# Audio-WestlakeU/FS-EEND

Hardware: AMD Instinct MI355X
Metric: audio frames/sec (T=500 chunks) (higher is better)
Workload: dtype bf16

## Files before the change

fs-eend_amd/csrc/api.hip:

```cpp
#include "../../include/eend_hip.h"
#include "kernels.h"
#include <stdlib.h>
#include <string.h>

namespace {
GemmParams base_params(const void* A, int lda, const void* W, int ldw, const float* bias, int M, int N, int K) {
    GemmParams p;
    memset(&p, 0, sizeof(p));
    p.A = A; p.lda = lda; p.W = W; p.ldw = ldw; p.bias = bias;
    p.M = M; p.N = N; p.K = K; p.ldo = N; p.Tp = 64; p.H = 4; p.dh = 64; p.C = 1;
    p.alpha = 1.0f; p.eps = 1e-5f; p.conv_cin = 64; p.conv_pad = 0; p.drop.scale = 1.0f;
#ifdef EEND_GEMM_ABLATE
    const char* d = getenv("EEND_GEMM_DBG");
    p.dbg = d ? atoi(d) : 0;
#endif
    return p;
}
}

extern "C" {

int eend_abi_version(void) { return 5; }

int eend_bn_cast_pad_f16(const float* x, const float* bn_weight, const float* bn_bias, const float* bn_mean,
// ... 207 lines not shown
    memset(&p, 0, sizeof(p));
    p.A = A; p.lda = lda; p.wstream = wstream; p.bo = bo; p.g1 = g1; p.be1 = be1; p.eps1 = eps1; p.res32 = res; p.res16 = res_f16;
    p.b1 = b1; p.b2 = b2; p.alpha = 1.0f; p.gamma = g2; p.beta = be2; p.eps = eps2; p.out32 = out_f32; p.out16 = out_f16;
    p.M = M; p.F = F;
    return ffn_stream_chunked(p, 1, 1, FFN_EPI_RES_LN, (hipStream_t)stream);
}

int eend_attnout_ffn_stream_lo_f16(const void* A, int lda, const void* wstream, const float* bo, const float* res, const float* g1,
                                   const float* be1, float eps1, const float* b1, const float* b2, const float* g2, const float* be2,
                                   float eps2, float* out_f32, void* out_f16, void* out_lo_f16, int M, int F, void* stream) {
    if (!res) return EEND_EINVAL;
    FfnStreamParams p;
    memset(&p, 0, sizeof(p));
    p.A = A; p.lda = lda; p.wstream = wstream; p.bo = bo; p.g1 = g1; p.be1 = be1; p.eps1 = eps1; p.res32 = res; p.wo_lo = 1;
    p.b1 = b1; p.b2 = b2; p.alpha = 1.0f; p.gamma = g2; p.beta = be2; p.eps = eps2; p.out32 = out_f32; p.out16 = out_f16; p.out16lo = out_lo_f16;
    p.M = M; p.F = F;
    return ffn_stream_chunked(p, 1, 1, FFN_EPI_RES_LN, (hipStream_t)stream);
}

int eend_conv_stream_elems(int ktaps) { return (int)eend_conv_stream_nelems(ktaps); }

int eend_conv_stream_ok(int cin, int ktaps, int pad) { return eend_conv_stream_supported(cin, ktaps, pad); }

int eend_conv_stream_pack_f16(const void* Wr, void* stream_out, int ktaps, void* stream) {
    return eend_launch_conv_stream_pack(Wr, stream_out, ktaps, (hipStream_t)stream);
}

int eend_conv1d_l2norm_stream_f16(const void* X, const void* wstream, const float* bias, const int* ilens, float* out_f32,
                                  void* out_f16, int nseq, int Tp, int ktaps, int pad, void* stream) {
    ConvStreamParams p;
    memset(&p, 0, sizeof(p));
    p.X = X; p.wstream = wstream; p.bias = bias; p.ilens = ilens; p.out32 = out_f32; p.out16 = out_f16; p.nseq = nseq; p.Tp = Tp;
    p.ktaps = ktaps; p.pad = pad;
    return eend_launch_conv_stream(p, (hipStream_t)stream);
}

int eend_encoder_input_ok(int Fin, int Tp, int ldw) { return eend_encin_supported(Fin, Tp, ldw); }

int eend_encoder_input_f16(const float* const* x_ptrs, const int* lens, float pad_value, const float* bn_w, const float* bn_b,
                           const float* bn_mean, const float* bn_var, float bn_eps, const void* W_f16, int ldw, const float* bias,
                           const float* gamma, const float* beta, float eps, float* out_f32, void* out_f16, int B, int T, int Tp,
                           int Fin, void* stream) {
    EncInParams p;
    memset(&p, 0, sizeof(p));
    p.x_ptrs = x_ptrs; p.lens = lens; p.pad_value = pad_value; p.bn_w = bn_w; p.bn_b = bn_b; p.bn_mean = bn_mean; p.bn_var = bn_var;
    p.bn_eps = bn_eps; p.W = W_f16; p.ldw = ldw; p.bias = bias; p.gamma = gamma; p.beta = beta; p.eps = eps; p.out32 = out_f32;
    p.out16 = out_f16; p.B = B; p.T = T; p.Tp = Tp; p.Fin = Fin;
    return eend_launch_encin(p, (hipStream_t)stream);
}

int eend_dec_stream_elems(int F) { return F >= 64 && F % 64 == 0 && F <= 2048 ? (int)eend_dec_stream_nelems(F) : 0; }

int eend_dec_stream_ok(int C, int Tp) { return eend_dec_stream_supported(C, Tp); }

int eend_dec_stream_pack_f16(const void* Wo1, const void* W_in, const void* Wo2, const void* W1, const void* W2, void* stream_out, int F,
                             void* stream) {
    return eend_launch_dec_stream_pack(Wo1, W_in, Wo2, W1, W2, stream_out, F, (hipStream_t)stream);
}

int eend_attnout_spk_ffn_stream_f16(const void* A, int lda, const void* wstream, const float* bo1, const void* res_f16, const float* g11,
                                    const float* be11, float eps11, const float* b_in, const float* bo2, const float* g21, const float* be21,
                                    float eps21, const float* b1, const float* b2, const float* g22, const float* be22, float eps22,
                                    void* out_f16, int B, int C, int Tp, int F, float scale, void* stream) {
    DecStreamParams p;
    memset(&p, 0, sizeof(p));
    p.A = A; p.lda = lda; p.wstream = wstream; p.bo1 = bo1; p.g11 = g11; p.be11 = be11; p.eps11 = eps11; p.res16 = res_f16; p.bin = b_in;
// ... 429 lines not shown
```

fs-eend_amd/csrc/conv_stream.hip:

```cpp
#include "common.h"
#include "kernels.h"
#include "wstream.h"

namespace {

constexpr int NR = 4;
constexpr int NF = 8;
constexpr int TM = 128, WM = 64;
constexpr int SLOT = STREAM_ITEM;
constexpr int NSLOT = 5;
constexpr int MAXTAPS = 24;
constexpr int XROWS = TM + MAXTAPS;
constexpr int L_RING = 0;
constexpr int L_X = NSLOT * SLOT;
constexpr int L_VEC = L_X + XROWS * 512;
constexpr int L_SS = L_VEC + 1024;
constexpr int SMEM = L_SS + 1024;
constexpr int NB = 8, PD = 4;
constexpr int INFL = 4 * (NSLOT - 3);

__global__ void conv_stream_pack_kernel(const _Float16* __restrict__ Wr, _Float16* __restrict__ out, int ktaps) {
    const long total = (long)ktaps * 8 * 1024;
    for (long t = (long)blockIdx.x * blockDim.x + threadIdx.x; t < total; t += (long)gridDim.x * blockDim.x) {
        const int item = (int)(t >> 10), w = (int)(t & 1023), i = w >> 6, l = w & 63, f = l & 15, g = l >> 4;
        const int tau = item >> 3, kc = item & 7;
        const _Float16* src = Wr + (size_t)((i >> 3) * 128 + (f >> 2) * 32 + (i & 7) * 4 + (f & 3)) * (ktaps * 256) + tau * 256 + kc * 32 + g * 8;
        _Float16* dst = out + t * 8;
#pragma unroll
        for (int e = 0; e < 8; ++e) dst[e] = src[e];
    }
}

__global__ __launch_bounds__(256, 1)
void conv_stream_kernel(const ConvStreamParams p) {
    const int S = p.ktaps * 8;
    const int TPS = (p.Tp + TM - 1) / TM;
    const int ntiles = p.nseq * TPS;
    const int xrows = TM + p.ktaps - 1;

    int tid = threadIdx.x;
    asm volatile("" : "+v"(tid));
    int lane = tid & 63;
    const int wave = __builtin_amdgcn_readfirstlane(tid >> 6);
    int frow = lane & 15, g = lane >> 4;

    WeightRing<NSLOT, L_RING> ring(p.wstream, S, wave, lane);
    ring.prime();
    float* vb = (float*)(smem + L_VEC);
    vb[tid] = p.bias[tid];

    auto stage_x = [&](int tile) __attribute__((always_inline)) {
        const int seq = __builtin_amdgcn_readfirstlane(tile / TPS), t0 = (tile - seq * TPS) * TM;
        int len = p.ilens[seq];
        len = len < p.Tp ? len : p.Tp;
        const __amdgpu_buffer_rsrc_t rx = __builtin_amdgcn_make_buffer_rsrc((void*)((const char*)p.X + (size_t)seq * p.Tp * 512), 0, len * 512, 0x00020000);
        const int npc = (xrows + 1) >> 1;
        for (int pc = wave; pc < npc; pc += 4) {
            const int r = 2 * pc + (lane >> 5);
            const int off = (t0 - p.pad + r) * 512 + (((lane & 31) ^ (r & 7)) << 4);
            __builtin_amdgcn_raw_ptr_buffer_load_lds(rx, (lds_char*)(smem + L_X + pc * 1024), 16, off, 0, 0, 0);
        }
    };

    const int rg = wave >> 1, nh = wave & 1;
    f16x8 wf[NB];
    f32x4 acc[NF][NR];
    bool cold = true;
    for (int tile = blockIdx.x; tile < ntiles; tile += gridDim.x) {
        asm volatile("" : "+v"(tid));
        lane = tid & 63; frow = lane & 15; g = lane >> 4;
        ring.set_lane(lane);
        const int seq = __builtin_amdgcn_readfirstlane(tile / TPS), t0 = (tile - seq * TPS) * TM;
        asm volatile("s_waitcnt lgkmcnt(0)\n\ts_barrier" ::: "memory");
        stage_x(tile);
        asm volatile("s_waitcnt vmcnt(0)\n\ts_barrier" ::: "memory");
#pragma unroll
        for (int i = 0; i < NF; ++i) {
            const f32x4 b4 = *(const f32x4*)(vb + nh * 128 + g * 32 + i * 4);
#pragma unroll
            for (int j = 0; j < NR; ++j) acc[i][j] = b4;
        }
        const char* xl = smem + L_X;
        auto read_x = [&](int q, f16x8 (&xo)[NR]) __attribute__((always_inline)) {
            const int tau = q >> 3, kc = q & 7;
#pragma unroll
            for (int j = 0; j < NR; ++j) {
                const int r = rg * WM + j * 16 + frow + tau;
                xo[j] = *(const f16x8*)(xl + r * 512 + (((kc * 4 + g) ^ (r & 7)) << 4));
            }
        };
        f16x8 xf[NR], xn[NR];
        read_x(0, xf);
        for (int q = 0; q < S; ++q) {
            if (q > 0) {
                wait_vm<INFL>();
                __builtin_amdgcn_s_barrier();
            }
            const char* wc = smem + L_RING + ring.slot * SLOT + nh * (NF * 1024) + lane * 16;
            const char* wn = smem + L_RING + ring.next_slot() * SLOT + nh * (NF * 1024) + lane * 16;
            const int sd = ring.refill_slot();
            if (cold) {
                sfor<PD>([&](auto Q) __attribute__((always_inline)) { wf[decltype(Q)::value % NB] = *(const f16x8*)(wc + decltype(Q)::value * 1024); });
                cold = false;
            }
            sfor<NF>([&](auto PI) __attribute__((always_inline)) {
                constexpr int pi = decltype(PI)::value;
                const f16x8 w = wf[pi % NB];
#pragma unroll
                for (int j = 0; j < NR; ++j) acc[pi][j] = __builtin_amdgcn_mfma_f32_16x16x32_f16(w, xf[j], acc[pi][j], 0, 0, 0);
                if constexpr (pi + PD < NF) wf[(pi + PD) % NB] = *(const f16x8*)(wc + (pi + PD) * 1024);
                else wf[(pi + PD) % NB] = *(const f16x8*)(wn + (pi + PD - NF) * 1024);
                if constexpr (pi < 4) ring.piece<pi>(sd);
                if constexpr (pi == 2) { if (q + 1 < S) read_x(q + 1, xn); }
                __builtin_amdgcn_sched_barrier(0);
            });
#pragma unroll
            for (int j = 0; j < NR; ++j) xf[j] = xn[j];
            ring.advance();
            ring.rotate();
        }
        asm volatile("s_waitcnt lgkmcnt(0)\n\ts_barrier" ::: "memory");
        asm volatile("" : "+v"(tid));
        lane = tid & 63; frow = lane & 15; g = lane >> 4;
        float* ssl = (float*)(smem + L_SS);
        float ss[NR];
#pragma unroll
        for (int j = 0; j < NR; ++j) {
            f32x2 sq2 = f32x2{0.f, 0.f};
#pragma unroll
            for (int i = 0; i < NF; ++i) {
                const f32x2 x0 = f32x2{acc[i][j][0], acc[i][j][1]}, x1 = f32x2{acc[i][j][2], acc[i][j][3]};
                sq2 = x1 * x1 + (x0 * x0 + sq2);
            }
            ss[j] = wave_g_allreduce_add(sq2[0] + sq2[1]);
            if (g == 0) ssl[(rg * WM + j * 16 + frow) * 2 + nh] = ss[j];
        }
        asm volatile("s_waitcnt lgkmcnt(0)\n\ts_barrier" ::: "memory");
        char* st = smem + L_X + wave * 4096;
        const int tlim = p.Tp - t0;
        sfor<NR>([&](auto J) __attribute__((always_inline)) {
            constexpr int j = decltype(J)::value;
            const float rinv = 1.0f / __builtin_sqrtf(ss[j] + ssl[(rg * WM + j * 16 + frow) * 2 + (nh ^ 1)]);
            if (p.inv_norm) { const int rr = rg * WM + j * 16 + frow; if (g == 0 && nh == 0 && rr < tlim) p.inv_norm[(size_t)seq * p.Tp + t0 + rr] = rinv; }
#pragma unroll
            for (int half = 0; half < 2; ++half) {
                const int rb = rg * WM + j * 16 + half * 8;
                if ((frow >> 3) == half) {
#pragma unroll
                    for (int e = 0; e < 4; ++e) {
                        f16x8 o;
#pragma unroll
                        for (int q = 0; q < 8; ++q) o[q] = to_f16_sat(acc[e * 2 + (q >> 2)][j][q & 3] * rinv);
                        *(f16x8*)(st + (frow & 7) * 256 + (((g * 4 + e) ^ (frow & 7)) << 4)) = o;
                    }
                }
                wave_lds_sync();
#pragma unroll
                for (int ps = 0; ps < 2; ++ps) {
                    const int rr = lane >> 3, cc = (lane & 7) + 8 * ps;
                    const f16x8 v = *(const f16x8*)(st + rr * 256 + ((cc ^ rr) << 4));
                    if (rb + rr < tlim) *(f16x8*)((_Float16*)p.out16 + ((size_t)seq * p.Tp + t0 + rb + rr) * 256 + nh * 128 + cc * 8) = v;
                }
                wave_lds_sync();
                if ((frow >> 3) == half) {
#pragma unroll
                    for (int e = 0; e < 8; ++e) *(f32x4*)(st + (frow & 7) * 512 + (((g * 8 + e) ^ (frow & 7)) << 4)) = acc[e][j] * rinv;
                }
                wave_lds_sync();
#pragma unroll
                for (int ps = 0; ps < 4; ++ps) {
                    const int rr = lane >> 3, cc = (lane & 7) + 8 * ps;
                    const f32x4 v = *(const f32x4*)(st + rr * 512 + ((cc ^ rr) << 4));
                    if (rb + rr < tlim) *(f32x4*)(p.out32 + ((size_t)seq * p.Tp + t0 + rb + rr) * 256 + nh * 128 + cc * 4) = v;
                }
                wave_lds_sync();
            }
        });
    }
    asm volatile("s_waitcnt vmcnt(0)" ::: "memory");
}

}

long eend_conv_stream_nelems(int ktaps) { return (long)ktaps * 8 * (SLOT / 2); }

int eend_conv_stream_supported(int cin, int ktaps, int pad) { return cin == 256 && ktaps >= 1 && ktaps <= MAXTAPS && pad >= 0 && pad < ktaps; }

int eend_launch_conv_stream_pack(const void* Wr, void* out, int ktaps, hipStream_t stream) {
    if (!Wr || !out || ktaps < 1 || ktaps > MAXTAPS) return EEND_EINVAL;
    hipLaunchKernelGGL(conv_stream_pack_kernel, dim3(ktaps * 8 * 4), dim3(256), 0, stream, (const _Float16*)Wr, (_Float16*)out, ktaps);
    return hipGetLastError() == hipSuccess ? EEND_OK : EEND_ELAUNCH;
}

int eend_launch_conv_stream(const ConvStreamParams& p, hipStream_t stream) {
    if (!p.X || !p.wstream || !p.bias || !p.ilens || !p.out32 || !p.out16 || p.nseq <= 0 || p.Tp <= 0 || !eend_conv_stream_supported(256, p.ktaps, p.pad) ||
        (long)p.Tp * 512 >= (1L << 31))
        return EEND_EINVAL;
    return stream_launch<conv_stream_kernel>(p, SMEM, p.nseq * ((p.Tp + TM - 1) / TM), eend_cu_count(), stream);
}
```

fs-eend_amd/csrc/kernels.h:

```cpp
#pragma once
#include <hip/hip_runtime.h>
#include <stdint.h>
#include "../../include/eend_hip.h"
#include "common.h"

enum GemmEpilogue {
    EPI_PLAIN_F16 = 0,
    EPI_PLAIN_RELU_F16 = 1,
    EPI_QK_HEADS = 2,
    EPI_VT_HEADS = 3,
    EPI_RES_LN = 4,
    EPI_L2NORM = 5,
    EPI_CONVERT = 6,
    EPI_RES_SCALE = 7,
    EPI_RES_SCALE_LN16 = 8,
    EPI_PLAIN_SWISH_F16 = 9,
    EPI_GLU_F16 = 10,
    EPI_QK_HEADS_F16 = 11,
    EPI_KTVT_HEADS_F16 = 12,
    EPI_PLAIN_BF16 = 13,
    EPI_MASK_BF16 = 14,
    EPI_F32_ROWMASK = 15,
    EPI_RES_LN_TRAIN = 16,
    EPI_L2NORM_TRAIN = 17,
// ... 313 lines not shown
    const float* be11;
    float eps11;
    const void* res16;
    const float* bin;
    const float* bo2;
    const float* g21;
    const float* be21;
    float eps21;
    const float* b1;
    const float* b2;
    const float* g22;
    const float* be22;
    float eps22;
    void* out16;
    int B, C, Tp, F;
    float scale;
};
long eend_dec_stream_nelems(int F);
int eend_dec_stream_supported(int C, int Tp);
int eend_launch_dec_stream_pack(const void* Wo1, const void* Win, const void* Wo2, const void* W1, const void* W2, void* out, int F,
                                hipStream_t stream);
int eend_launch_dec_stream(const DecStreamParams& p, hipStream_t stream);
int eend_launch_convert_fanout_rows(const void* E, const void* W1, const float* pc, float* out32, void* out16, int B, int Tp, int C,
                                    hipStream_t stream);
struct ConvStreamParams {
    const void* X;
    const void* wstream;
    const float* bias;
    const int* ilens;
    float* out32;
    void* out16;
    float* inv_norm;
    int nseq, Tp, ktaps, pad;
};
long eend_conv_stream_nelems(int ktaps);
int eend_conv_stream_supported(int cin, int ktaps, int pad);
int eend_launch_conv_stream_pack(const void* Wr, void* out, int ktaps, hipStream_t stream);
int eend_launch_conv_stream(const ConvStreamParams& p, hipStream_t stream);
struct EncInParams {
    const float* const* x_ptrs;
    const int* lens;
    float pad_value;
    const float *bn_w, *bn_b, *bn_mean, *bn_var;
    float bn_eps;
    const void* W;
    int ldw;
    const float *bias, *gamma, *beta;
    float eps;
    float* out32;
    void* out16;
    int B, T, Tp, Fin;
};
int eend_encin_supported(int Fin, int Tp, int ldw);
int eend_launch_encin(const EncInParams& p, hipStream_t stream);
int eend_launch_convert_fanout_f32(const float* emb, const float* W, int ldw, const float* pc, float* out32, void* out16, void* out16lo,
                                   int B, int Tp, int C, hipStream_t stream);
int eend_launch_attn_causal_full(const AttnParams& p, hipStream_t stream);

enum ProjKind { PROJ_ROWMAJOR = 0, PROJ_HEADS = 1, PROJ_HEADS_T = 2, PROJ_HEADS_BOTH = 3 };
struct ProjParams {
    const void* X;
    const void* W;
    const float* bias;
    int M, N, ldx, Tp, H;
    int kind[4];
    int is_bf16[4];
    void* out[4];
    void* out2[4];
    int ld[4];
};
// ... 156 lines not shown
```

fs-eend_amd/fs_model.py:

```python
import copy
import math
from typing import List, Optional, Sequence

import torch
import torch.nn as nn
from torch import Tensor

from . import ops
from .lib import EendHipError

_D_SUPPORTED = 256
_H_SUPPORTED = 4


class PositionalEncoding(nn.Module):

    def __init__(self, d_model, dropout=0.1, max_len=5000):
        super().__init__()
        self.dropout = nn.Dropout(p=dropout)
        pe = torch.zeros(max_len, d_model)
        position = torch.arange(0, max_len, dtype=torch.float).unsqueeze(1)
        div_term = torch.exp(torch.arange(0, d_model, 2).float() * (-math.log(10000.0) / d_model))
        pe[:, 0::2] = torch.sin(position * div_term)
        pe[:, 1::2] = torch.cos(position * div_term)
        self.register_buffer("pe", pe.unsqueeze(0))


class TransformerEncoder(nn.Module):

    def __init__(self, encoder_layer, num_layers, norm=None):
        super().__init__()
        self.layers = nn.ModuleList([copy.deepcopy(encoder_layer) for _ in range(num_layers)])
        self.num_layers = num_layers
        self.norm = norm
# ... 162 lines not shown
        P = {}
        enc = self.enc
        Fin = enc.in_size
        Fin_pad = (Fin + 63) // 64 * 64
        w = torch.zeros(enc.n_units, Fin_pad, dtype=torch.float16, device=dev)
        w[:, :Fin] = enc.encoder.weight.detach().to(torch.float16)
        P["enc.in.w"], P["enc.in.b"] = w, _f32(enc.encoder.bias)
        P["enc.in.g"], P["enc.in.beta"] = _f32(enc.encoder_norm.weight), _f32(enc.encoder_norm.bias)
        P["enc.in.eps"] = enc.encoder_norm.eps
        P["bn"] = tuple(_f32(t) for t in (enc.bn.weight, enc.bn.bias, enc.bn.running_mean, enc.bn.running_var))
        P["bn.eps"] = enc.bn.eps
        P["Fin_pad"] = Fin_pad
        layers = []
        for l in enc.transformer_encoder.layers:
            layers.append(dict(
                in_w=_f16(_qscaled(l.self_attn.in_proj_weight)), in_b=_f32(_qscaled(l.self_attn.in_proj_bias)),
                out_w=_f16(l.self_attn.out_proj.weight), out_b=_f32(l.self_attn.out_proj.bias),
                w1=_f16(l.linear1.weight), b1=_f32(l.linear1.bias), w2=_f16(l.linear2.weight), b2=_f32(l.linear2.bias),
                g1=_f32(l.norm1.weight), be1=_f32(l.norm1.bias), eps1=l.norm1.eps,
                g2=_f32(l.norm2.weight), be2=_f32(l.norm2.bias), eps2=l.norm2.eps))
        for L in layers:
            if ops.stream_ok(L["w1"].shape[0]):
                L["ws"] = ops.ffn_stream_pack(L["out_w"], L["w1"], L["w2"])
            L["in_wp"] = ops.inproj_attn_pack(L["in_w"])
        P["enc.layers"] = layers
        cw = self.cnn.weight.detach()
        P["cnn.w"] = cw.permute(0, 2, 1).reshape(cw.shape[0], -1).to(torch.float16).contiguous()
        P["cnn.b"] = _f32(self.cnn.bias)
        P["cnn.k"], P["cnn.pad"] = cw.shape[2], self.cnn.padding[0]
        if ops.conv_stream_ok(cw.shape[1], cw.shape[2], self.cnn.padding[0]) and cw.shape[0] == 256:
            P["cnn.ws"] = ops.conv_stream_pack(P["cnn.w"], cw.shape[2])
        D = enc.n_units
        P["convert.w1"] = _f16(self.dec.convert.weight[:, :D])
        dl = []
        for l in self.dec.attractor_decoder.layers:
            dl.append(dict(
                in1_w=_f16(_qscaled(l.self_attn1.in_proj_weight)), in1_b=_f32(_qscaled(l.self_attn1.in_proj_bias)),
                out1_w=_f16(l.self_attn1.out_proj.weight), out1_b=_f32(l.self_attn1.out_proj.bias),
                in2_w=_f16(l.self_attn2.in_proj_weight), in2_b=_f32(l.self_attn2.in_proj_bias),
                out2_w=_f16(l.self_attn2.out_proj.weight), out2_b=_f32(l.self_attn2.out_proj.bias),
                w1=_f16(l.linear1.weight), b1=_f32(l.linear1.bias), w2=_f16(l.linear2.weight), b2=_f32(l.linear2.bias),
                g11=_f32(l.norm11.weight), be11=_f32(l.norm11.bias), eps11=l.norm11.eps,
                g21=_f32(l.norm21.weight), be21=_f32(l.norm21.bias), eps21=l.norm21.eps,
                g22=_f32(l.norm22.weight), be22=_f32(l.norm22.bias), eps22=l.norm22.eps))
        for L in dl:
            if ops.stream_ok(L["w1"].shape[0]):
                L["ws"] = ops.ffn_stream_pack(L["out2_w"], L["w1"], L["w2"])
            L["ws1"] = ops.spk_stream_pack(L["out1_w"], L["in2_w"])
            if ops.stream_ok(L["w1"].shape[0]):
                L["wsd"] = ops.dec_stream_pack(L["out1_w"], L["in2_w"], L["out2_w"], L["w1"], L["w2"])
            L["in1_wp"] = ops.inproj_attn_pack(L["in1_w"])
        P["dec.layers"] = dl
        self._prep, self._prep_key = P, key
        self._pc = {}
        return P

    def _convert_const(self, C):
        if C not in self._pc:
            from . import lib as _lib
            D = self.enc.n_units if hasattr(self.enc, "n_units") else self.n_units
            dev = self.dec.convert.weight.device
            W = self.dec.convert.weight.detach().to(torch.float32).contiguous()
            b = self.dec.convert.bias.detach().to(torch.float32).contiguous()
            pe = self.dec.pos_enc.pe[0, :C].to(device=dev, dtype=torch.float32).contiguous()
            pc = torch.empty(C, D, dtype=torch.float32, device=dev)
            L = _lib.load()
# ... 38 lines not shown
            ops.linear_res_ln(ws.xin16, P["enc.in.w"], P["enc.in.b"], None, P["enc.in.g"], P["enc.in.beta"], None, ws.h16, P["enc.in.eps"])
        o16 = ws.o16[:Me]

        def time_attention(x16, Ly, wkey, bkey, nseq, delay, kv):
            o = ws.o16[:nseq * Tp]
            if Tp <= 512:
                ops.inproj_attn_causal_packed(x16, Ly[wkey + "p"], Ly[bkey], o, nseq, H, Tp, delay, kv)
                return o
            need = ops.inproj_attn_long_scratch(nseq, Tp, delay, kv) if Tp <= 3072 else None
            if need is not None:
                if ws.attn_part.numel() < need[0]:
                    ws.attn_part = torch.empty(need[0], dtype=torch.float16, device=o.device)
                if ws.attn_lse.numel() < need[1]:
                    ws.attn_lse = torch.empty(need[1], dtype=torch.float32, device=o.device)
                ops.inproj_attn_causal_long(x16, Ly[wkey + "p"], Ly[bkey], o, ws.attn_part, ws.attn_lse, nseq, H, Tp, delay, kv)
            else:
                n = nseq * Tp * D
                if ws.q is None:
                    ws.q, ws.k, ws.vt = (torch.empty(ws.Mx * ws.D, dtype=torch.bfloat16, device=o.device) for _ in range(3))
                ops.inproj_heads(x16, Ly[wkey], Ly[bkey], ws.q[:n], ws.k[:n], ws.vt[:n], nseq, Tp, H)
                ops.attn_causal(ws.q[:n], ws.k[:n], ws.vt[:n], o, nseq, H, Tp, delay, kv, scale=ops.LN2)
            return o

        for L in P["enc.layers"]:
            time_attention(ws.h16, L, "in_w", "in_b", B, delay_e, kv_e)
            if "ws" in L:
                ops.attnout_ffn_stream(o16, L["ws"], L["out_b"], None, ws.h16, L["g1"], L["be1"], L["eps1"], L["b1"], L["b2"], L["g2"],
                                       L["be2"], L["eps2"], None, ws.h16)
            else:
                ops.attnout_ffn_fused_res16(o16, L["out_w"], L["out_b"], ws.h16, L["g1"], L["be1"], L["eps1"], L["w1"], L["b1"],
                                            L["w2"], L["b2"], L["g2"], L["be2"], L["eps2"], None, ws.h16)

        emb32 = torch.empty(Me, D, dtype=torch.float32, device=dev)
        if "cnn.ws" in P:
            ops.conv1d_l2norm_stream(ws.h16, P["cnn.ws"], P["cnn.b"], il, emb32, ws.emb16, B, Tp, P["cnn.k"], P["cnn.pad"])
        else:
            ops.conv1d_l2norm(ws.h16, P["cnn.w"], P["cnn.b"], il, emb32, ws.emb16, B, Tp, D, P["cnn.k"], P["cnn.pad"])

        ops.convert_fanout(ws.emb16, P["convert.w1"], self._convert_const(C), None, ws.a16, B, Tp, C)
        o16 = ws.o16[:Md]
        for L in P["dec.layers"]:
            time_attention(ws.a16, L, "in1_w", "in1_b", B * C, self.dec.mask_delay, T)
            if "wsd" in L and ops.dec_stream_ok(C, Tp):
                ops.attnout_spk_ffn_stream(o16, L["wsd"], L["out1_b"], ws.a16, L["g11"], L["be11"], L["eps11"], L["in2_b"], L["out2_b"],
                                           L["g21"], L["be21"], L["eps21"], L["b1"], L["b2"], L["g22"], L["be22"], L["eps22"], ws.a16, B, C, Tp)
                continue
            ops.attnout_spk_stream(o16, L["ws1"], L["out1_b"], ws.a16, L["g11"], L["be11"], L["eps11"], ws.a16, L["in2_b"], o16, B, C, Tp)
            if "ws" in L:
                ops.attnout_ffn_stream(o16, L["ws"], L["out2_b"], None, ws.a16, L["g21"], L["be21"], L["eps21"], L["b1"], L["b2"],
                                       L["g22"], L["be22"], L["eps22"], None, ws.a16)
            else:
                ops.attnout_ffn_fused_res16(o16, L["out2_w"], L["out2_b"], ws.a16, L["g21"], L["be21"], L["eps21"], L["w1"], L["b1"],
                                            L["w2"], L["b2"], L["g22"], L["be22"], L["eps22"], None, ws.a16)

        attr = torch.empty(B, T, C, D, dtype=torch.float32, device=dev)
        logits = torch.empty(B, T, C, dtype=torch.float32, device=dev)
        ops.head_l2dot(emb32, ws.a16, attr, logits, B, T, Tp, C, D)
        emb = emb32.view(B, Tp, D)
        return logits, emb, attr, T, Tp

    @torch.no_grad()
    def test(self, src, ilens, max_nspks=6):
        logits, emb, attr, T, Tp = self._run(src, ilens, max_nspks)
        output = [logits[b, :l] for b, l in enumerate(ilens)]
        embs = [emb[b, :l] for b, l in enumerate(ilens)]
        attractors = [attr[b, :l] for b, l in enumerate(ilens)]
        return output, embs, attractors

    def forward(self, src, tgt, ilens):
        if torch.is_grad_enabled() and any(p.requires_grad for p in self.parameters()):
            from .autograd import fs_forward_with_grad
            return fs_forward_with_grad(self, src, tgt, ilens)
# ... 12 lines not shown
```

fs-eend_amd/lib.py:

```python
import ctypes
import os

_HERE = os.path.dirname(os.path.abspath(__file__))
LIB_PATH = os.environ.get("EEND_HIP_LIB") or os.path.join(_HERE, "csrc", "libeend_hip.so")

_vp, _i, _f = ctypes.c_void_p, ctypes.c_int, ctypes.c_float
_l = ctypes.c_long

ABI_VERSION = 5

PROTOTYPES = {
    "eend_abi_version": [],
    "eend_bn_cast_pad_f16": [_vp, _vp, _vp, _vp, _vp, _f, _vp, _i, _i, _i, _i, _i, _i, _vp],
    "eend_gather_bn_cast_pad_f16": [_vp, _vp, _f, _vp, _vp, _vp, _vp, _f, _vp, _i, _i, _i, _i, _i, _i, _vp],
    "eend_linear_f16": [_vp, _i, _vp, _i, _vp, _vp, _i, _i, _i, _i, _i, _vp],
    "eend_inproj_heads_bf16": [_vp, _i, _vp, _i, _vp, _vp, _vp, _vp, _i, _i, _i, _i, _i, _vp],
    "eend_linear_glu_f16": [_vp, _i, _vp, _i, _vp, _vp, _i, _i, _i, _i, _vp],
    "eend_linear_res_ln_f16": [_vp, _i, _vp, _i, _vp, _vp, _f, _vp, _vp, _f, _vp, _vp, _i, _i, _vp],
    "eend_linear_res16_ln_f16": [_vp, _i, _vp, _i, _vp, _vp, _f, _vp, _vp, _f, _vp, _vp, _i, _i, _vp],
    "eend_linear_res_scale_ln16_f16": [_vp, _i, _vp, _i, _vp, _vp, _f, _vp, _vp, _f, _vp, _vp, _i, _i, _vp],
    "eend_ffn_fused_f16": [_vp, _i, _vp, _vp, _vp, _vp, _vp, _f, _vp, _vp, _f, _vp, _vp, _i, _i, _i, _i, _vp],
    "eend_attnout_ffn_fused_f16": [_vp, _i, _vp, _vp, _vp, _vp, _vp, _f, _vp, _vp, _vp, _vp, _vp, _vp, _f, _vp, _vp, _vp, _vp, _i, _i, _vp],
    "eend_attnout_ffn_fused_res16_f16": [_vp, _i, _vp, _vp, _vp, _vp, _vp, _f, _vp, _vp, _vp, _vp, _vp, _vp, _f, _vp, _vp, _i, _i, _vp],
    "eend_convert_fanout_f32": [_vp, _vp, _i, _vp, _vp, _vp, _vp, _i, _i, _i, _vp],
    "eend_ffn_stream_elems": [_i, _i],
    "eend_ffn_stream_pack_f16": [_vp, _vp, _vp, _vp, _i, _vp],
    "eend_ffn_stream_pack_lo_f16": [_vp, _vp, _vp, _vp, _vp, _i, _vp],
    "eend_attnout_ffn_stream_lo_f16": [_vp, _i, _vp, _vp, _vp, _vp, _vp, _f, _vp, _vp, _vp, _vp, _f, _vp, _vp, _vp, _i, _i, _vp],
    "eend_ffn_stream_f16": [_vp, _i, _vp, _vp, _vp, _vp, _f, _vp, _vp, _f, _vp, _vp, _i, _i, _i, _i, _vp],
    "eend_conv_stream_elems": [_i],
    "eend_conv_stream_ok": [_i, _i, _i],
    "eend_conv_stream_pack_f16": [_vp, _vp, _i, _vp],
    "eend_conv1d_l2norm_stream_f16": [_vp, _vp, _vp, _vp, _vp, _vp, _i, _i, _i, _i, _vp],
    "eend_encoder_input_ok": [_i, _i, _i],
    "eend_encoder_input_f16": [_vp, _vp, _f, _vp, _vp, _vp, _vp, _f, _vp, _i, _vp, _vp, _vp, _f, _vp, _vp, _i, _i, _i, _i, _vp],
    "eend_inproj_attn_packed_elems": [],
    "eend_inproj_attn_pack_f16": [_vp, _vp, _vp],
    "eend_inproj_attn_causal_packed_f16": [_vp, _i, _vp, _vp, _vp, _i, _i, _i, _i, _i, _i, _vp],
    "eend_inproj_attn_train_bf16": [_vp, _i, _vp, _vp, _vp, _i, _vp, _vp, _vp, _vp, _i, _i, _i, _i, _i, _vp, _vp],
    "eend_gemm_acc_stream_elems": [_i],
    "eend_gemm_acc_stream_ok": [_i, _i, _i],
    "eend_gemm_acc_stream_pack_bf16": [_vp, _i, _vp, _i, _vp],
    "eend_gemm_acc_stream_bf16": [_vp, _i, _vp, _vp, _i, _i, _vp],
    "eend_proj_stream_elems": [_i],
    "eend_proj_stream_pack_f16": [_vp, _vp, _i, _vp],
    "eend_proj_stream_ok": [_i, _i, _i, _i, _i, _vp],
    "eend_proj_stream_f16": [_vp, _i, _vp, _vp, _i, _i, _i, _i, _vp, _vp],
    "eend_inproj_attn_long_scratch_elems": [_i, _i, _i, _i, _vp, _vp],
    "eend_inproj_attn_causal_long_f16": [_vp, _i, _vp, _vp, _vp, _vp, _vp, _i, _i, _i, _i, _i, _i, _vp],
    "eend_spk_stream_elems": [],
    "eend_spk_stream_ok": [_i, _i],
    "eend_spk_stream_pack_f16": [_vp, _vp, _vp, _vp],
    "eend_attnout_spk_stream_f16": [_vp, _i, _vp, _vp, _vp, _vp, _vp, _f, _vp, _vp, _vp, _i, _i, _i, _f, _vp],
    "eend_attnout_spk_stream_res32_f16": [_vp, _i, _vp, _vp, _vp, _vp, _vp, _f, _vp, _vp, _vp, _i, _i, _i, _f, _vp],
    "eend_dec_stream_elems": [_i],
    "eend_dec_stream_ok": [_i, _i],
    "eend_dec_stream_pack_f16": [_vp, _vp, _vp, _vp, _vp, _vp, _i, _vp],
    "eend_attnout_spk_ffn_stream_f16": [_vp, _i, _vp, _vp, _vp, _vp, _vp, _f, _vp, _vp, _vp, _vp, _f, _vp, _vp, _vp, _vp, _f, _vp, _i, _i, _i,
                                        _i, _f, _vp],
    "eend_ffn_stream_max_rows": [_i],
    "eend_debug_ffn_stream_set": [_i, _l],
    "eend_attnout_ffn_stream_f16": [_vp, _i, _vp, _vp, _vp, _vp, _vp, _vp, _f, _vp, _vp, _vp, _vp, _f, _vp, _vp, _i, _i, _vp],
    "eend_emb_consistency_f32": [_vp, _vp, _vp, _f, _vp, _vp, _i, _i, _i, _i, _i, _vp],
    "eend_activity_median_u8": [_vp, _i, _i, _i, _f, _i, _vp, _vp],
    "eend_activity_segments_i32": [_vp, _i, _i, _vp, _vp, _i, _vp],
    "eend_der_counters_u64": [_vp, _i, _vp, _i, _i, _i, _i, _vp, _vp],
# ... 157 lines not shown
```

fs-eend_amd/ops.py:

```python
import math

import torch

from . import lib as _lib

F16, BF16, F32 = torch.float16, torch.bfloat16, torch.float32


def _stream():
    return torch.cuda.current_stream().cuda_stream


def _p(t):
    return None if t is None else t.data_ptr()


def _chk(t, dtype, name):
    if t is None:
        return
    if not t.is_cuda:
        raise _lib.EendHipError(f"{name}: expected a GPU tensor (the HIP path has no CPU fallback)")
    if t.dtype != dtype:
        raise _lib.EendHipError(f"{name}: expected {dtype}, got {t.dtype}")
    if not t.is_contiguous():
# ... 183 lines not shown
def conv1d_l2norm(x16, wr16, bias, ilens_i32, out32, out16, nseq, Tp, cin, ktaps, pad):
    L = _lib.load()
    _chk(x16, F16, "x16"); _chk(wr16, F16, "wr16"); _chk(bias, F32, "bias"); _chk(ilens_i32, torch.int32, "ilens")
    _chk(out32, F32, "out32"); _chk(out16, F16, "out16")
    _lib.check(L.eend_conv1d_l2norm_f16(_p(x16), _p(wr16), _p(bias), _p(ilens_i32), _p(out32), _p(out16), nseq,
                                        Tp, cin, ktaps, pad, _stream()), "eend_conv1d_l2norm_f16")


def conv_stream_ok(cin, ktaps, pad):
    return bool(_lib.load().eend_conv_stream_ok(int(cin), int(ktaps), int(pad)))


def conv_stream_pack(wr16, ktaps):
    L = _lib.load()
    _chk(wr16, F16, "wr16")
    if wr16.shape != (256, ktaps * 256):
        raise _lib.EendHipError("conv_stream_pack: expected Wr [256][ktaps*256]")
    out = torch.empty(L.eend_conv_stream_elems(int(ktaps)), dtype=F16, device=wr16.device)
    _lib.check(L.eend_conv_stream_pack_f16(_p(wr16), _p(out), int(ktaps), _stream()), "eend_conv_stream_pack_f16")
    return out


def conv1d_l2norm_stream(x16, wstream, bias, ilens_i32, out32, out16, nseq, Tp, ktaps, pad):
    L = _lib.load()
    _chk(x16, F16, "x16"); _chk(wstream, F16, "wstream"); _chk(bias, F32, "bias"); _chk(ilens_i32, torch.int32, "ilens")
    _chk(out32, F32, "out32"); _chk(out16, F16, "out16")
    if x16.shape != (nseq * Tp, 256) or out32.shape != (nseq * Tp, 256) or out16.shape != (nseq * Tp, 256) or \
            wstream.numel() != L.eend_conv_stream_elems(int(ktaps)):
        raise _lib.EendHipError("conv1d_l2norm_stream: shape mismatch")
    _lib.check(L.eend_conv1d_l2norm_stream_f16(_p(x16), _p(wstream), _p(bias), _p(ilens_i32), _p(out32), _p(out16), nseq, Tp, ktaps, pad,
                                               _stream()), "eend_conv1d_l2norm_stream_f16")


def convert_fanout(e16, w1_16, pc, out32, out16, B, Tp, C):
    L = _lib.load()
    _chk(e16, F16, "e16"); _chk(w1_16, F16, "w1"); _chk(pc, F32, "pc"); _chk(out32, F32, "out32"); _chk(out16, F16, "out16")
    _lib.check(L.eend_convert_fanout_f16(_p(e16), _p(w1_16), _p(pc), _p(out32), _p(out16), B, Tp, C, _stream()),
               "eend_convert_fanout_f16")


def convert_fanout_f32(e32, w32, pc, out32, out16, B, Tp, C, out16lo=None):
    L = _lib.load()
    _chk(e32, F32, "e32"); _chk(w32, F32, "w32"); _chk(pc, F32, "pc"); _chk(out32, F32, "out32"); _chk(out16, F16, "out16"); _chk(out16lo, F16, "out16lo")
    _lib.check(L.eend_convert_fanout_f32(_p(e32), _p(w32), w32.stride(0), _p(pc), _p(out32), _p(out16), _p(out16lo), B, Tp, C, _stream()),
               "eend_convert_fanout_f32")


LN2 = math.log(2.0)
QSCALE_LOG2 = (1.0 / math.sqrt(64.0)) * math.log2(math.e)


def attn_causal(q, k, vt, o16, nseq, H, Tp, mask_delay=0, kv_len=None, scale=1.0 / math.sqrt(64.0)):
    L = _lib.load()
    _chk(q, BF16, "q"); _chk(k, BF16, "k"); _chk(vt, BF16, "vt"); _chk(o16, F16, "o16")
    _lib.check(L.eend_attn_causal_bf16(_p(q), _p(k), _p(vt), _p(o16), nseq, H, Tp, o16.stride(0), mask_delay,
                                       Tp if kv_len is None else kv_len, scale, _stream()), "eend_attn_causal_bf16")


def inproj_attn_pack(w_in):
    L = _lib.load()
    _chk(w_in, F16, "w_in")
    if w_in.shape != (768, 256):
        raise _lib.EendHipError("inproj_attn_pack: expected in_proj_weight [768][256]")
    out = torch.empty(L.eend_inproj_attn_packed_elems(), dtype=F16, device=w_in.device)
    _lib.check(L.eend_inproj_attn_pack_f16(_p(w_in), _p(out), _stream()), "eend_inproj_attn_pack_f16")
    return out
# ... 714 lines not shown
```

include/eend_hip.h:

```cpp
#ifndef EEND_HIP_H
#define EEND_HIP_H

#ifdef __cplusplus
extern "C" {
#endif

#define EEND_OK 0
#define EEND_EINVAL (-1)
#define EEND_ELAUNCH (-2)

#define EEND_ABI_VERSION 5
int eend_abi_version(void);

int eend_bn_cast_pad_f16(const float* x, const float* bn_weight, const float* bn_bias,
                         const float* bn_mean, const float* bn_var, float eps, void* out_f16,
                         int B, int T, int Tp, int Fin, int Fpad, int apply_bn, void* stream);

int eend_gather_bn_cast_pad_f16(const void* const* x_ptrs, const int* lens, float pad_value,
                                const float* bn_weight, const float* bn_bias, const float* bn_mean,
                                const float* bn_var, float eps, void* out_f16, int B, int T, int Tp, int Fin,
                                int Fpad, int apply_bn, void* stream);

int eend_encoder_input_ok(int Fin, int Tp, int ldw);
int eend_encoder_input_f16(const float* const* x_ptrs, const int* lens, float pad_value, const float* bn_w, const float* bn_b,
// ... 1 lines not shown
                           const float* gamma, const float* beta, float eps, float* out_f32, void* out_f16, int B, int T, int Tp,
                           int Fin, void* stream);

int eend_linear_f16(const void* A, int lda, const void* W, int ldw, const float* bias, void* out_f16,
                    int ldo, int M, int N, int K, int act, void* stream);

int eend_linear_glu_f16(const void* A, int lda, const void* Wi, int ldw, const float* bias_i, void* out_f16,
                        int ldo, int M, int N2, int K, void* stream);

int eend_inproj_heads_bf16(const void* A, int lda, const void* W, int ldw, const float* bias, void* Q_bf16,
                           void* K_bf16, void* Vt_bf16, int nseq, int Tp, int H, int dh, int K, void* stream);

int eend_linear_res_ln_f16(const void* A, int lda, const void* W, int ldw, const float* bias,
                           const float* res, float alpha, const float* gamma, const float* beta, float eps,
                           float* out_f32, void* out_f16, int M, int K, void* stream);

int eend_linear_res_scale_ln16_f16(const void* A, int lda, const void* W, int ldw, const float* bias,
                                   const float* res, float alpha, const float* gamma, const float* beta,
                                   float eps, float* out_f32, void* out_f16, int M, int K, void* stream);

int eend_linear_res_scale_f16(const void* A, int lda, const void* W, int ldw, const float* bias,
                              const float* res, float alpha, float* out_f32, void* out_f16, int M, int K,
                              void* stream);

int eend_conv1d_l2norm_f16(const void* X, const void* Wr, const float* bias, const int* ilens,
                           float* out_f32, void* out_f16, int nseq, int Tp, int cin, int ktaps, int pad,
                           void* stream);

int eend_conv_stream_elems(int ktaps);
int eend_conv_stream_ok(int cin, int ktaps, int pad);
int eend_conv_stream_pack_f16(const void* Wr, void* stream_out, int ktaps, void* stream);
int eend_conv1d_l2norm_stream_f16(const void* X, const void* wstream, const float* bias, const int* ilens, float* out_f32,
                                  void* out_f16, int nseq, int Tp, int ktaps, int pad, void* stream);

int eend_convert_fanout_f16(const void* E, const void* W1, const float* pc, float* out_f32, void* out_f16,
                            int B, int Tp, int C, void* stream);
int eend_convert_fanout_f32(const float* E_f32, const float* W_f32, int ldw, const float* pc, float* out_f32, void* out_f16,
                            void* out_lo_f16, int B, int Tp, int C, void* stream);

int eend_attn_causal_bf16(const void* Q, const void* K, const void* Vt, void* O_f16, int nseq, int H,
                          int Tp, int ldo, int mask_delay, int kv_len, float scale, void* stream);

int eend_ffn_fused_f16(const void* X, int ldx, const void* W1, const float* b1, const void* W2, const float* b2,
                       const float* res, float alpha, const float* gamma, const float* beta, float eps,
                       float* out_f32, void* out_f16, int M, int F, int act, int residual_stream_unnormalised,
                       void* stream);

int eend_attnout_ffn_fused_f16(const void* A, int lda, const void* Wo, const float* bo, const float* res,
                               const float* g1, const float* be1, float eps1, const void* W1, const float* b1,
                               const void* W2, const float* b2, const float* g2, const float* be2, float eps2,
                               float* out_f32, void* out_f16, void* out_lo_f16, const void* Wo_lo, int M, int F, void* stream);
int eend_linear_res16_ln_f16(const void* A, int lda, const void* W, int ldw, const float* bias, const void* res_f16,
                             float alpha, const float* gamma, const float* beta, float eps, float* out_f32,
                             void* out_f16, int M, int K, void* stream);
int eend_attnout_ffn_fused_res16_f16(const void* A, int lda, const void* Wo, const float* bo, const void* res_f16,
                                     const float* g1, const float* be1, float eps1, const void* W1, const float* b1,
                                     const void* W2, const float* b2, const float* g2, const float* be2, float eps2,
                                     float* out_f32, void* out_f16, int M, int F, void* stream);

int eend_ffn_stream_max_rows(int lda);
int eend_debug_ffn_stream_set(int tile_fragments, long max_rows_per_launch);

int eend_ffn_stream_elems(int F, int with_wo);
int eend_ffn_stream_pack_f16(const void* Wo, const void* W1, const void* W2, void* stream_out, int F, void* stream);
int eend_ffn_stream_f16(const void* X, int ldx, const void* wstream, const float* b1, const float* b2,
                        const float* res, float alpha, const float* gamma, const float* beta, float eps,
// ... 359 lines not shown
```

Baseline: 17.04 million.

## Fuse convert fan-out projection into streamed conv1d L2-norm kernel

Adds a templated FANOUT variant of the streamed conv kernel. After the L2 normalisation it writes the normalised embedding tile to LDS and runs eight extra weight-ring items using the packed convert.w1 weights. It then writes the C fanned-out copies, each with its per-attractor constant added, directly to the decoder input buffer. This removes the separate convert_fanout launch and its re-read of the embedding from global memory. In exchange the conv kernel gets a longer tail per tile, more registers for the fan accumulators, and C extra store passes.

```diff
diff --git a/fs-eend_amd/csrc/api.hip b/fs-eend_amd/csrc/api.hip
--- a/fs-eend_amd/csrc/api.hip
+++ b/fs-eend_amd/csrc/api.hip
@@ -263,6 +263,25 @@
     memset(&p, 0, sizeof(p));
     p.X = X; p.wstream = wstream; p.bias = bias; p.ilens = ilens; p.out32 = out_f32; p.out16 = out_f16; p.nseq = nseq; p.Tp = Tp;
     p.ktaps = ktaps; p.pad = pad;
+    return eend_launch_conv_stream(p, (hipStream_t)stream);
+}
+
+int eend_conv_fanout_stream_elems(int ktaps) { return (int)eend_conv_fanout_stream_nelems(ktaps); }
+
+int eend_conv_fanout_stream_ok(int cin, int ktaps, int pad, int C) { return eend_conv_fanout_stream_supported(cin, ktaps, pad, C); }
+
+int eend_conv_fanout_stream_pack_f16(const void* Wr, const void* W1, void* stream_out, int ktaps, void* stream) {
+    return eend_launch_conv_fanout_stream_pack(Wr, W1, stream_out, ktaps, (hipStream_t)stream);
+}
+
+int eend_conv1d_l2norm_fanout_stream_f16(const void* X, const void* wstream, const float* bias, const int* ilens, const float* pc,
+                                         float* out_f32, void* out_f16, void* fan_f16, int nseq, int Tp, int ktaps, int pad, int C,
+                                         void* stream) {
+    if (!fan_f16 || !pc) return EEND_EINVAL;
+    ConvStreamParams p;
+    memset(&p, 0, sizeof(p));
+    p.X = X; p.wstream = wstream; p.bias = bias; p.ilens = ilens; p.out32 = out_f32; p.out16 = out_f16; p.nseq = nseq; p.Tp = Tp;
+    p.ktaps = ktaps; p.pad = pad; p.fan16 = fan_f16; p.pc = pc; p.C = C;
     return eend_launch_conv_stream(p, (hipStream_t)stream);
 }
 
diff --git a/fs-eend_amd/csrc/conv_stream.hip b/fs-eend_amd/csrc/conv_stream.hip
--- a/fs-eend_amd/csrc/conv_stream.hip
+++ b/fs-eend_amd/csrc/conv_stream.hip
@@ -31,6 +31,46 @@
     }
 }
 
+#define CONV_STREAM_ITEMS(NITEMS, ACC)                                                                                                  \
+    {                                                                                                                                   \
+        f16x8 xf[NR], xn[NR];                                                                                                           \
+        read_x(0, xf);                                                                                                                  \
+        for (int q = 0; q < (NITEMS); ++q) {                                                                                            \
+             \
+             \
+            if (q > 0) {                                                                                                                \
+                wait_vm<INFL>();                                                                                                        \
+                __builtin_amdgcn_s_barrier();                                                                                           \
+            }                                                                                                                           \
+             \
+             \
+            const char* wc = smem + L_RING + ring.slot * SLOT + nh * (NF * 1024) + lane * 16;                                           \
+            const char* wn = smem + L_RING + ring.next_slot() * SLOT + nh * (NF * 1024) + lane * 16;                                    \
+            const int sd = ring.refill_slot();                                                                                          \
+            if (cold) {                                                                                                                 \
+                sfor<PD>([&](auto Q) __attribute__((always_inline)) {                                                                   \
+                    wf[decltype(Q)::value % NB] = *(const f16x8*)(wc + decltype(Q)::value * 1024);                                      \
+                });                                                                                                                     \
+                cold = false;                                                                                                           \
+            }                                                                                                                           \
+            sfor<NF>([&](auto PI) __attribute__((always_inline)) {                                                                      \
+                constexpr int pi = decltype(PI)::value;                                                                                 \
+                const f16x8 w = wf[pi % NB];                                                                                            \
+                _Pragma("unroll") for (int j = 0; j < NR; ++j)                                                                          \
+                    ACC[pi][j] = __builtin_amdgcn_mfma_f32_16x16x32_f16(w, xf[j], ACC[pi][j], 0, 0, 0);                                 \
+                if constexpr (pi + PD < NF) wf[(pi + PD) % NB] = *(const f16x8*)(wc + (pi + PD) * 1024);                                \
+                else wf[(pi + PD) % NB] = *(const f16x8*)(wn + (pi + PD - NF) * 1024);                                                  \
+                if constexpr (pi < 4) ring.piece<pi>(sd);                                                                               \
+                if constexpr (pi == 2) { if (q + 1 < (NITEMS)) read_x(q + 1, xn); }                                                     \
+                __builtin_amdgcn_sched_barrier(0);                                                                                      \
+            });                                                                                                                         \
+            _Pragma("unroll") for (int j = 0; j < NR; ++j) xf[j] = xn[j];                                                               \
+            ring.advance();                                                                                                             \
+            ring.rotate();                                                                                                              \
+        }                                                                                                                               \
+    }
+
+template <bool FANOUT>
 __global__ __launch_bounds__(256, 1)
 void conv_stream_kernel(const ConvStreamParams p) {
     const int S = p.ktaps * 8;
@@ -44,7 +84,7 @@
     const int wave = __builtin_amdgcn_readfirstlane(tid >> 6);
     int frow = lane & 15, g = lane >> 4;
 
-    WeightRing<NSLOT, L_RING> ring(p.wstream, S, wave, lane);
+    WeightRing<NSLOT, L_RING> ring(p.wstream, FANOUT ? S + 8 : S, wave, lane);
     ring.prime();
     float* vb = (float*)(smem + L_VEC);
     vb[tid] = p.bias[tid];
@@ -89,36 +129,7 @@
                 xo[j] = *(const f16x8*)(xl + r * 512 + (((kc * 4 + g) ^ (r & 7)) << 4));
             }
         };
-        f16x8 xf[NR], xn[NR];
-        read_x(0, xf);
-        for (int q = 0; q < S; ++q) {
-            if (q > 0) {
-                wait_vm<INFL>();
-                __builtin_amdgcn_s_barrier();
-            }
-            const char* wc = smem + L_RING + ring.slot * SLOT + nh * (NF * 1024) + lane * 16;
-            const char* wn = smem + L_RING + ring.next_slot() * SLOT + nh * (NF * 1024) + lane * 16;
-            const int sd = ring.refill_slot();
-            if (cold) {
-                sfor<PD>([&](auto Q) __attribute__((always_inline)) { wf[decltype(Q)::value % NB] = *(const f16x8*)(wc + decltype(Q)::value * 1024); });
-                cold = false;
-            }
-            sfor<NF>([&](auto PI) __attribute__((always_inline)) {
-                constexpr int pi = decltype(PI)::value;
-                const f16x8 w = wf[pi % NB];
-#pragma unroll
-                for (int j = 0; j < NR; ++j) acc[pi][j] = __builtin_amdgcn_mfma_f32_16x16x32_f16(w, xf[j], acc[pi][j], 0, 0, 0);
-                if constexpr (pi + PD < NF) wf[(pi + PD) % NB] = *(const f16x8*)(wc + (pi + PD) * 1024);
-                else wf[(pi + PD) % NB] = *(const f16x8*)(wn + (pi + PD - NF) * 1024);
-                if constexpr (pi < 4) ring.piece<pi>(sd);
-                if constexpr (pi == 2) { if (q + 1 < S) read_x(q + 1, xn); }
-                __builtin_amdgcn_sched_barrier(0);
-            });
-#pragma unroll
-            for (int j = 0; j < NR; ++j) xf[j] = xn[j];
-            ring.advance();
-            ring.rotate();
-        }
+        CONV_STREAM_ITEMS(S, acc)
         asm volatile("s_waitcnt lgkmcnt(0)\n\ts_barrier" ::: "memory");
         asm volatile("" : "+v"(tid));
         lane = tid & 63; frow = lane & 15; g = lane >> 4;
@@ -136,11 +147,39 @@
             if (g == 0) ssl[(rg * WM + j * 16 + frow) * 2 + nh] = ss[j];
         }
         asm volatile("s_waitcnt lgkmcnt(0)\n\ts_barrier" ::: "memory");
+        float rv[FANOUT ? NR : 1];
+        f32x4 fan[FANOUT ? NF : 1][FANOUT ? NR : 1];
+        if constexpr (FANOUT) {
+#pragma unroll
+            for (int j = 0; j < NR; ++j) {
+                const int r = rg * WM + j * 16 + frow;
+                rv[j] = 1.0f / __builtin_sqrtf(ss[j] + ssl[r * 2 + (nh ^ 1)]);
+#pragma unroll
+                for (int e = 0; e < 4; ++e) {
+                    f16x8 o;
+#pragma unroll
+                    for (int q = 0; q < 8; ++q) o[q] = to_f16_sat(acc[e * 2 + (q >> 2)][j][q & 3] * rv[j]);
+                    *(f16x8*)(smem + L_X + r * 512 + (((nh * 16 + g * 4 + e) ^ (r & 7)) << 4)) = o;
+                }
+            }
+#pragma unroll
+            for (int i = 0; i < NF; ++i)
+#pragma unroll
+                for (int j = 0; j < NR; ++j) fan[i][j] = f32x4{0.f, 0.f, 0.f, 0.f};
+            wait_vm_lgkm0<INFL>();
+            __builtin_amdgcn_s_barrier();
+            CONV_STREAM_ITEMS(8, fan)
+            asm volatile("s_waitcnt lgkmcnt(0)\n\ts_barrier" ::: "memory");
+            asm volatile("" : "+v"(tid));
+            lane = tid & 63; frow = lane & 15; g = lane >> 4;
+        }
         char* st = smem + L_X + wave * 4096;
         const int tlim = p.Tp - t0;
         sfor<NR>([&](auto J) __attribute__((always_inline)) {
             constexpr int j = decltype(J)::value;
-            const float rinv = 1.0f / __builtin_sqrtf(ss[j] + ssl[(rg * WM + j * 16 + frow) * 2 + (nh ^ 1)]);
+            float rinv;
+            if constexpr (FANOUT) rinv = rv[j];
+            else rinv = 1.0f / __builtin_sqrtf(ss[j] + ssl[(rg * WM + j * 16 + frow) * 2 + (nh ^ 1)]);
             if (p.inv_norm) { const int rr = rg * WM + j * 16 + frow; if (g == 0 && nh == 0 && rr < tlim) p.inv_norm[(size_t)seq * p.Tp + t0 + rr] = rinv; }
 #pragma unroll
             for (int half = 0; half < 2; ++half) {
@@ -176,13 +215,56 @@
                 wave_lds_sync();
             }
         });
+        if constexpr (FANOUT) {
+            for (int c = 0; c < p.C; ++c) {
+                f32x4 pcv[NF];
+#pragma unroll
+                for (int i = 0; i < NF; ++i) pcv[i] = *(const f32x4*)(p.pc + c * 256 + nh * 128 + g * 32 + i * 4);
+                const __amdgpu_buffer_rsrc_t ro = __builtin_amdgcn_make_buffer_rsrc(
+                    (void*)((char*)p.fan16 + ((size_t)seq * p.C + c) * p.Tp * 512), 0, p.Tp * 512, 0x00020000);
+                sfor<NR>([&](auto J) __attribute__((always_inline)) {
+                    constexpr int j = decltype(J)::value;
+#pragma unroll
+                    for (int e = 0; e < 4; ++e) {
+                        f16x8 o;
+#pragma unroll
+                        for (int q = 0; q < 8; ++q) o[q] = to_f16_sat(fan[e * 2 + (q >> 2)][j][q & 3] + pcv[e * 2 + (q >> 2)][q & 3]);
+                        *(f16x8*)(st + frow * 256 + (((g * 4 + e) ^ frow) << 4)) = o;
+                    }
+                    wave_lds_sync();
+#pragma unroll
+                    for (int ps = 0; ps < 4; ++ps) {
+                        const int rr = (lane >> 4) + 4 * ps, cc = lane & 15;
+                        const f16x8 v = *(const f16x8*)(st + rr * 256 + ((cc ^ rr) << 4));
+                        __builtin_amdgcn_raw_buffer_store_b128(__builtin_bit_cast(u32x4, v), ro,
+                                                               (t0 + rg * WM + j * 16 + rr) * 512 + nh * 256 + cc * 16, 0, 0);
+                    }
+                    wave_lds_sync();
+                });
+            }
+        }
     }
     asm volatile("s_waitcnt vmcnt(0)" ::: "memory");
 }
 
+#undef CONV_STREAM_ITEMS
+
 }
 
 long eend_conv_stream_nelems(int ktaps) { return (long)ktaps * 8 * (SLOT / 2); }
+
+long eend_conv_fanout_stream_nelems(int ktaps) { return (long)(ktaps * 8 + 8) * (SLOT / 2); }
+
+int eend_conv_fanout_stream_supported(int cin, int ktaps, int pad, int C) {
+    return eend_conv_stream_supported(cin, ktaps, pad) && C >= 1 && C <= 12;
+}
+
+int eend_launch_conv_fanout_stream_pack(const void* Wr, const void* W1, void* out, int ktaps, hipStream_t stream) {
+    if (!W1) return EEND_EINVAL;
+    const int rc = eend_launch_conv_stream_pack(Wr, out, ktaps, stream);
+    if (rc != EEND_OK) return rc;
+    return eend_launch_conv_stream_pack(W1, (_Float16*)out + eend_conv_stream_nelems(ktaps), 1, stream);
+}
 
 int eend_conv_stream_supported(int cin, int ktaps, int pad) { return cin == 256 && ktaps >= 1 && ktaps <= MAXTAPS && pad >= 0 && pad < ktaps; }
 
@@ -196,5 +278,9 @@
     if (!p.X || !p.wstream || !p.bias || !p.ilens || !p.out32 || !p.out16 || p.nseq <= 0 || p.Tp <= 0 || !eend_conv_stream_supported(256, p.ktaps, p.pad) ||
         (long)p.Tp * 512 >= (1L << 31))
         return EEND_EINVAL;
-    return stream_launch<conv_stream_kernel>(p, SMEM, p.nseq * ((p.Tp + TM - 1) / TM), eend_cu_count(), stream);
-}
+    if (p.fan16) {
+        if (!p.pc || p.inv_norm || !eend_conv_fanout_stream_supported(256, p.ktaps, p.pad, p.C)) return EEND_EINVAL;
+        return stream_launch<conv_stream_kernel<true>>(p, SMEM, p.nseq * ((p.Tp + TM - 1) / TM), eend_cu_count(), stream);
+    }
+    return stream_launch<conv_stream_kernel<false>>(p, SMEM, p.nseq * ((p.Tp + TM - 1) / TM), eend_cu_count(), stream);
+}
diff --git a/fs-eend_amd/csrc/kernels.h b/fs-eend_amd/csrc/kernels.h
--- a/fs-eend_amd/csrc/kernels.h
+++ b/fs-eend_amd/csrc/kernels.h
@@ -369,10 +369,16 @@
     void* out16;
     float* inv_norm;
     int nseq, Tp, ktaps, pad;
+    void* fan16;
+    const float* pc;
+    int C;
 };
 long eend_conv_stream_nelems(int ktaps);
 int eend_conv_stream_supported(int cin, int ktaps, int pad);
 int eend_launch_conv_stream_pack(const void* Wr, void* out, int ktaps, hipStream_t stream);
+long eend_conv_fanout_stream_nelems(int ktaps);
+int eend_conv_fanout_stream_supported(int cin, int ktaps, int pad, int C);
+int eend_launch_conv_fanout_stream_pack(const void* Wr, const void* W1, void* out, int ktaps, hipStream_t stream);
 int eend_launch_conv_stream(const ConvStreamParams& p, hipStream_t stream);
 struct EncInParams {
     const float* const* x_ptrs;
diff --git a/fs-eend_amd/fs_model.py b/fs-eend_amd/fs_model.py
--- a/fs-eend_amd/fs_model.py
+++ b/fs-eend_amd/fs_model.py
@@ -1,5 +1,6 @@
 import copy
 import math
+import os
 from typing import List, Optional, Sequence
 
 import torch
@@ -228,6 +229,8 @@
             P["cnn.ws"] = ops.conv_stream_pack(P["cnn.w"], cw.shape[2])
         D = enc.n_units
         P["convert.w1"] = _f16(self.dec.convert.weight[:, :D])
+        if "cnn.ws" in P and D == 256:
+            P["cnn.wsf"] = ops.conv_fanout_stream_pack(P["cnn.w"], P["convert.w1"], cw.shape[2])
         dl = []
         for l in self.dec.attractor_decoder.layers:
             dl.append(dict(
@@ -332,12 +335,17 @@
                                             L["w2"], L["b2"], L["g2"], L["be2"], L["eps2"], None, ws.h16)
 
         emb32 = torch.empty(Me, D, dtype=torch.float32, device=dev)
-        if "cnn.ws" in P:
-            ops.conv1d_l2norm_stream(ws.h16, P["cnn.ws"], P["cnn.b"], il, emb32, ws.emb16, B, Tp, P["cnn.k"], P["cnn.pad"])
+        fused_tail = os.environ.get("EEND_FS_FUSED_TAIL", "1") != "0"
+        if fused_tail and "cnn.wsf" in P and ops.conv_fanout_stream_ok(D, P["cnn.k"], P["cnn.pad"], C):
+            ops.conv1d_l2norm_fanout_stream(ws.h16, P["cnn.wsf"], P["cnn.b"], il, self._convert_const(C), emb32, ws.emb16, ws.a16,
+                                            B, Tp, P["cnn.k"], P["cnn.pad"], C)
         else:
-            ops.conv1d_l2norm(ws.h16, P["cnn.w"], P["cnn.b"], il, emb32, ws.emb16, B, Tp, D, P["cnn.k"], P["cnn.pad"])
-
-        ops.convert_fanout(ws.emb16, P["convert.w1"], self._convert_const(C), None, ws.a16, B, Tp, C)
+            if "cnn.ws" in P:
+                ops.conv1d_l2norm_stream(ws.h16, P["cnn.ws"], P["cnn.b"], il, emb32, ws.emb16, B, Tp, P["cnn.k"], P["cnn.pad"])
+            else:
+                ops.conv1d_l2norm(ws.h16, P["cnn.w"], P["cnn.b"], il, emb32, ws.emb16, B, Tp, D, P["cnn.k"], P["cnn.pad"])
+            ops.convert_fanout(ws.emb16, P["convert.w1"], self._convert_const(C), None, ws.a16, B, Tp, C)
+
         o16 = ws.o16[:Md]
         for L in P["dec.layers"]:
             time_attention(ws.a16, L, "in1_w", "in1_b", B * C, self.dec.mask_delay, T)
diff --git a/fs-eend_amd/lib.py b/fs-eend_amd/lib.py
--- a/fs-eend_amd/lib.py
+++ b/fs-eend_amd/lib.py
@@ -32,6 +32,10 @@
     "eend_conv_stream_ok": [_i, _i, _i],
     "eend_conv_stream_pack_f16": [_vp, _vp, _i, _vp],
     "eend_conv1d_l2norm_stream_f16": [_vp, _vp, _vp, _vp, _vp, _vp, _i, _i, _i, _i, _vp],
+    "eend_conv_fanout_stream_elems": [_i],
+    "eend_conv_fanout_stream_ok": [_i, _i, _i, _i],
+    "eend_conv_fanout_stream_pack_f16": [_vp, _vp, _vp, _i, _vp],
+    "eend_conv1d_l2norm_fanout_stream_f16": [_vp, _vp, _vp, _vp, _vp, _vp, _vp, _vp, _i, _i, _i, _i, _i, _vp],
     "eend_encoder_input_ok": [_i, _i, _i],
     "eend_encoder_input_f16": [_vp, _vp, _f, _vp, _vp, _vp, _vp, _f, _vp, _i, _vp, _vp, _vp, _f, _vp, _vp, _i, _i, _i, _i, _vp],
     "eend_inproj_attn_packed_elems": [],
diff --git a/fs-eend_amd/ops.py b/fs-eend_amd/ops.py
--- a/fs-eend_amd/ops.py
+++ b/fs-eend_amd/ops.py
@@ -239,6 +239,32 @@
                                                _stream()), "eend_conv1d_l2norm_stream_f16")
 
 
+def conv_fanout_stream_ok(cin, ktaps, pad, C):
+    return bool(_lib.load().eend_conv_fanout_stream_ok(int(cin), int(ktaps), int(pad), int(C)))
+
+
+def conv_fanout_stream_pack(wr16, w1_16, ktaps):
+    L = _lib.load()
+    _chk(wr16, F16, "wr16"); _chk(w1_16, F16, "w1")
+    if wr16.shape != (256, ktaps * 256) or w1_16.shape != (256, 256) or not w1_16.is_contiguous():
+        raise _lib.EendHipError("conv_fanout_stream_pack: expected Wr [256][ktaps*256] and a contiguous W1 [256][256]")
+    out = torch.empty(L.eend_conv_fanout_stream_elems(int(ktaps)), dtype=F16, device=wr16.device)
+    _lib.check(L.eend_conv_fanout_stream_pack_f16(_p(wr16), _p(w1_16), _p(out), int(ktaps), _stream()), "eend_conv_fanout_stream_pack_f16")
+    return out
+
+
+def conv1d_l2norm_fanout_stream(x16, wstream, bias, ilens_i32, pc, out32, out16, fan16, nseq, Tp, ktaps, pad, C):
+    L = _lib.load()
+    _chk(x16, F16, "x16"); _chk(wstream, F16, "wstream"); _chk(bias, F32, "bias"); _chk(ilens_i32, torch.int32, "ilens")
+    _chk(pc, F32, "pc"); _chk(out32, F32, "out32"); _chk(out16, F16, "out16"); _chk(fan16, F16, "fan16")
+    if x16.shape != (nseq * Tp, 256) or out32.shape != (nseq * Tp, 256) or out16.shape != (nseq * Tp, 256) or \
+            fan16.shape != (nseq * C * Tp, 256) or pc.shape != (C, 256) or wstream.numel() != L.eend_conv_fanout_stream_elems(int(ktaps)):
+        raise _lib.EendHipError("conv1d_l2norm_fanout_stream: shape mismatch")
+    _lib.check(L.eend_conv1d_l2norm_fanout_stream_f16(_p(x16), _p(wstream), _p(bias), _p(ilens_i32), _p(pc), _p(out32), _p(out16),
+                                                      _p(fan16), nseq, Tp, ktaps, pad, C, _stream()),
+               "eend_conv1d_l2norm_fanout_stream_f16")
+
+
 def convert_fanout(e16, w1_16, pc, out32, out16, B, Tp, C):
     L = _lib.load()
     _chk(e16, F16, "e16"); _chk(w1_16, F16, "w1"); _chk(pc, F32, "pc"); _chk(out32, F32, "out32"); _chk(out16, F16, "out16")
diff --git a/include/eend_hip.h b/include/eend_hip.h
--- a/include/eend_hip.h
+++ b/include/eend_hip.h
@@ -57,6 +57,12 @@
 int eend_conv_stream_pack_f16(const void* Wr, void* stream_out, int ktaps, void* stream);
 int eend_conv1d_l2norm_stream_f16(const void* X, const void* wstream, const float* bias, const int* ilens, float* out_f32,
                                   void* out_f16, int nseq, int Tp, int ktaps, int pad, void* stream);
+int eend_conv_fanout_stream_elems(int ktaps);
+int eend_conv_fanout_stream_ok(int cin, int ktaps, int pad, int C);
+int eend_conv_fanout_stream_pack_f16(const void* Wr, const void* W1, void* stream_out, int ktaps, void* stream);
+int eend_conv1d_l2norm_fanout_stream_f16(const void* X, const void* wstream, const float* bias, const int* ilens, const float* pc,
+                                         float* out_f32, void* out_f16, void* fan_f16, int nseq, int Tp, int ktaps, int pad, int C,
+                                         void* stream);
 
 int eend_convert_fanout_f16(const void* E, const void* W1, const float* pc, float* out_f32, void* out_f16,
                             int B, int Tp, int C, void* stream);
```

Result: no change. 17.04 million (-0.0%).
